# chrischoy/DeepGlobalRegistration

Hardware: AMD Instinct MI355X
Metric: pair registrations/sec (FCGF x2 + 1-NN + 6-D inlier net + gate + weighted Procrustes + SE(3) refinement) (higher is better)
Workload: dtype f32 results via 2 x f16 split operands (3 f16 MFMA products per MAC, f32 accumulate); k = 1 convs, kNN re-evaluation and registration in exact f32, SVD in f64

## Files before the change

### deepglobalregistration_amd/csrc/conv_os.hip

```cpp
#include <stdlib.h>

#include <type_traits>

#include "dgr_internal.h"
#include "split.h"

#ifdef DGR_OS_STAGE_CLK
__device__ unsigned long long dgr_os_stage_clk[8];
#define DGR_OS_CLK(i) do { if (threadIdx.x == 0) { const unsigned long long t_ = __builtin_amdgcn_s_memrealtime(); atomicAdd(&dgr_os_stage_clk[i], t_ - t_prev); t_prev = t_; } } while (0)
extern "C" int dgr_debug_os_stage_clk(unsigned long long *out8, int reset) {
  if (out8 && hipMemcpyFromSymbol(out8, HIP_SYMBOL(dgr_os_stage_clk), 8 * sizeof(unsigned long long)) != hipSuccess) return -1;
  if (reset) { unsigned long long z[8] = {0, 0, 0, 0, 0, 0, 0, 0}; if (hipMemcpyToSymbol(HIP_SYMBOL(dgr_os_stage_clk), z, sizeof(z)) != hipSuccess) return -1; }
  return 0;
}
#else
#define DGR_OS_CLK(i) do { } while (0)
#endif
struct ConvOsArgs {
  const float *in;
  float *out;
  const float *w16, *shift, *res;
  const uint4 *wb3;
  int64_t piece_stride;
  const int32_t *nbr, *n_out_dev;
  int64_t n_pad;
  int in_ld, in_relu, out_ld, out_relu, res_ld, res_relu;
  int cin, cout, nb16;
  const uint32_t *row_amax;
  float w_unscale;
  uint32_t *out_amax, *out_amax2;
};

template <int CP, int CS, int MB, int CK, int TM, int PM, int GW>
__global__ void __launch_bounds__(CS * 4 * (TM / 16 / GW)) sparse_conv_os(ConvOsArgs a) {
  constexpr bool BF3 = PM != 0;
  static_assert(PM == 0 || PM == 2, "arithmetic mode");
  constexpr int NP = PM == 0 ? 1 : 2;
  constexpr int GP = TM / 16;
  constexpr int NCW = CS / 16;
  constexpr int NWR = GP / GW;
  static_assert(GP % GW == 0, "groups per wave must divide the groups per tile");
  constexpr int NW = NCW * NWR;
  constexpr int THREADS = 64 * NW;
  constexpr int KV = 27;
  constexpr int PPT = CP / CK;
  constexpr int LDA = CK + 4, LDC = CS + 4;
  constexpr int C4K = CK / 4;
  constexpr int NCH = (TM * C4K + THREADS - 1) / THREADS;
  constexpr bool PIECE_GUARD = TM * C4K % THREADS != 0;
  constexpr int G = CK / 16;
  constexpr int GT = CP / 16;
  constexpr int KPW = (KV + NW - 1) / NW;
  constexpr int NGMAX = KV * ((MB / 16 + GP - 1) / GP * GP) + GP;
  static_assert(CP % CK == 0, "shape");
  constexpr int LDP = CK + 8;
  constexpr int PLANE = TM * LDP;
  constexpr int G32 = CK / 32;
  constexpr int ABYTES = BF3 ? 2 * NP * PLANE * 2 : 2 * TM * LDA * 4;
  __shared__ __attribute__((aligned(16))) char abuf[ABYTES];
  float (*As)[TM][LDA] = reinterpret_cast<float (*)[TM][LDA]>(abuf);
  unsigned short *Ps = reinterpret_cast<unsigned short *>(abuf);
  __shared__ __attribute__((aligned(16))) float acc_s[MB][LDC];
  __shared__ int in_idx[KV][MB];
  __shared__ float in_scale[PM == 2 ? KV : 1][MB];
  __shared__ unsigned char out_loc[KV][MB];
  __shared__ int cnt[KV];
  __shared__ int grp[NGMAX + GP];
  __shared__ int n_grp;

  const int tid = threadIdx.x;
  const int lane = tid & 63;
  const int wave = __builtin_amdgcn_readfirstlane(tid >> 6);
  const int cw = wave % NCW;
  const int rb0 = (wave / NCW) * GW;
  const int n_out = *a.n_out_dev;
  const int nblocks = (n_out + MB - 1) / MB;
  const int per = (nblocks + 7) >> 3;
  const int j = blockIdx.x >> 3;
  const int blk = (blockIdx.x & 7) * per + j;
  if (j >= per || blk >= nblocks) return;
  const int slice = blockIdx.y;
  const int64_t row0 = (int64_t)blk * MB;
#ifdef DGR_OS_STAGE_CLK
  unsigned long long t_prev = __builtin_amdgcn_s_memrealtime();
#endif

  if constexpr (PM == 2)
    for (int e = tid; e < KV * MB; e += THREADS) (&in_scale[0][0])[e] = 1.f;
  __syncthreads();
  {
    int v[KPW];
#pragma unroll
    for (int u = 0; u < KPW; ++u) {
      const int k = wave + u * NW;
      v[u] = (k < KV && lane < MB) ? a.nbr[(int64_t)k * a.n_pad + row0 + lane] : -1;
    }
#pragma unroll
    for (int u = 0; u < KPW; ++u) {
      const int k = wave + u * NW;
      if (k < KV) {
        const unsigned long long m = __ballot(v[u] >= 0);
        if (v[u] >= 0) {
          const int pos = __popcll(m & ((1ull << lane) - 1ull));
          in_idx[k][pos] = v[u];
          out_loc[k][pos] = (unsigned char)lane;
          if constexpr (PM == 2) in_scale[k][pos] = dgr_row_scale_of(a.row_amax[v[u]]);
        }
        if (lane == 0) cnt[k] = __popcll(m);
      }
    }
  }
  DGR_OS_CLK(0);
  for (int e = tid; e < MB * (CS / 4); e += THREADS) {
    const int r = e / (CS / 4), c = (e % (CS / 4)) * 4;
    f32x4 v = a.shift ? *reinterpret_cast<const f32x4 *>(a.shift + slice * CS + c) : f32x4{0.f, 0.f, 0.f, 0.f};
    if (a.res && row0 + r < n_out) {
      f32x4 x = *reinterpret_cast<const f32x4 *>(a.res + (row0 + r) * a.res_ld + slice * CS + c);
// ... 105 lines not shown
#pragma unroll
      for (int g = 0; g < G32; ++g) {
        const f16x8 ah = __builtin_bit_cast(f16x8, *reinterpret_cast<const uint4 *>(prow + 32 * g));
        const f16x8 am = __builtin_bit_cast(f16x8, *reinterpret_cast<const uint4 *>(prow + PLANE + 32 * g));
        const f16x8 wh = __builtin_bit_cast(f16x8, w[u].v[2 * g]), wm = __builtin_bit_cast(f16x8, w[u].v[2 * g + 1]);
        acc[u] = __builtin_amdgcn_mfma_f32_16x16x32_f16(wm, ah, acc[u], 0, 0, 0);
        acc[u] = __builtin_amdgcn_mfma_f32_16x16x32_f16(wh, am, acc[u], 0, 0, 0);
        acc[u] = __builtin_amdgcn_mfma_f32_16x16x32_f16(wh, ah, acc[u], 0, 0, 0);
      }
    }
  };
  if (NQ > 0) {
    gather(0);
#pragma unroll
    for (int u = 0; u < GW; ++u) wstep(0, u, w[u]);
    land(0);
    gather(NQ > 1 ? 1 : 0);
  }
  __syncthreads();

  for (int q = 0; q < NQ; ++q) {
    const int t = q / PPT, h = q % PPT;
    land(q + 1);
    gather(min(q + 2, NQ - 1));
    if (PPT == 1 || h == 0) {
#pragma unroll
      for (int u = 0; u < GW; ++u) acc[u] = f32x4{0.f, 0.f, 0.f, 0.f};
    }
#pragma unroll
    for (int u = 0; u < GW; ++u) {
      const int n_rows = __builtin_amdgcn_readfirstlane(grp[GP * t + rb0 + u]) >> 16;
      __builtin_amdgcn_sched_barrier(0);
      if (u == 0 || n_rows > 0) mfma_group(u, q & 1);
      wstep(q + 1, u, w[u]);
    }
    if (PPT == 1 || h == PPT - 1) {
#pragma unroll
      for (int u = 0; u < GW; ++u) {
        const int info = grp[GP * t + rb0 + u];
        if ((lane & 15) < (info >> 16)) {
          const int e = ((info >> 8) & 255) + (lane & 15);
          float *p = &acc_s[out_loc[info & 255][e]][16 * cw + 4 * (lane >> 4)];
          f32x4 v = *reinterpret_cast<f32x4 *>(p);
          if constexpr (PM == 2) {
            const float f = __builtin_bit_cast(float, 0x7f000000u - __builtin_bit_cast(uint32_t, in_scale[info & 255][e])) * a.w_unscale;
            v += acc[u] * f;
          } else {
            v += acc[u];
          }
          *reinterpret_cast<f32x4 *>(p) = v;
        }
      }
    }
    __syncthreads();
  }
  DGR_OS_CLK(2);
#ifdef DGR_OS_STAGE_CLK
  if (threadIdx.x == 0) { atomicAdd(&dgr_os_stage_clk[4], 1ull); atomicAdd(&dgr_os_stage_clk[5], (unsigned long long)NQ); }
#endif
  const float out_lo = a.out_relu ? 0.f : -__builtin_inff();
  static_assert(MB * (CS / 4) % THREADS == 0 || THREADS % (CS / 4) == 0, "row lanes stay inside a wave");
  for (int e0 = 0; e0 < MB * (CS / 4); e0 += THREADS) {
    const int e = e0 + tid;
    const bool live = e < MB * (CS / 4);
    const int r = live ? e / (CS / 4) : 0, c = (e % (CS / 4)) * 4;
    uint32_t mx = 0;
    if (live && row0 + r < n_out) {
      f32x4 v = *reinterpret_cast<const f32x4 *>(&acc_s[r][c]);
      v.x = fmaxf(v.x, out_lo); v.y = fmaxf(v.y, out_lo); v.z = fmaxf(v.z, out_lo); v.w = fmaxf(v.w, out_lo);
      *reinterpret_cast<f32x4 *>(a.out + (row0 + r) * a.out_ld + slice * CS + c) = v;
      mx = dgr_abs_max4(__builtin_bit_cast(i32x4, v));
    }
    if (a.out_amax || a.out_amax2) {
      mx = dgr_lane_max<CS / 4>(mx);
      if (live && (e % (CS / 4)) == 0 && row0 + r < n_out) {
        if (a.out_amax) atomicMax(a.out_amax + row0 + r, mx);
        if (a.out_amax2) atomicMax(a.out_amax2 + row0 + r, mx);
      }
    }
  }
  DGR_OS_CLK(3);
}

template <int CP, int CS, int MB, int CK, int TM>
static int launch_os(const ConvOsArgs &ka, int64_t n_out_cap, hipStream_t stream) {
  constexpr int GW = (MB >= 64 && CP <= 64) ? 1 : TM / 16;
  int64_t blocks = dgr_ceil_div(n_out_cap, MB);
  blocks = (blocks + 7) / 8 * 8;
  dim3 grid((unsigned)blocks, (unsigned)(ka.cout / CS));
  constexpr int threads = CS * 4 * (TM / 16 / GW);
  if (ka.wb3 && ka.row_amax)
    sparse_conv_os<CP, CS, MB, CK, TM, 2, GW><<<grid, threads, 0, stream>>>(ka);
  else
    sparse_conv_os<CP, CS, MB, CK, TM, 0, GW><<<grid, threads, 0, stream>>>(ka);
  DGR_LAUNCH_CHECK();
  return DGR_OK;
}

int dgr_conv_os_launch(const DgrConvOsLaunch &a, hipStream_t stream, const char **kernel_name) {
  if (a.dense) return dgr_conv_dense_launch(a, stream, kernel_name);
  if (a.up) return dgr_conv_up_launch(a, stream, kernel_name);
  DGR_REQUIRE(a.nbr && a.nbr->built && a.nbr->K == 27, "output-stationary conv: no neighbour table");
  DGR_REQUIRE((a.cin & 3) == 0 && (a.in_ld & 3) == 0 && (a.out_ld & 3) == 0 && (a.res == nullptr || (a.res_ld & 3) == 0),
              "output-stationary conv: channel counts and row strides must be multiples of 4");
  DGR_REQUIRE(a.cout % 32 == 0 && a.cin == a.cin_pad, "output-stationary conv: Cin = %d, Cout = %d must be multiples of 32",
              a.cin, a.cout);
  DGR_REQUIRE(a.n_in_cap > 0 && a.n_in_cap * (int64_t)a.in_ld < (1ll << 32) / 4 * 4,
              "output-stationary conv: input tensor beyond 32-bit element offsets");
  ConvOsArgs ka;
  ka.in = a.in; ka.out = a.out; ka.w16 = a.w16; ka.shift = a.shift; ka.res = a.res;
  ka.wb3 = dgr_exact_f32() ? nullptr : static_cast<const uint4 *>(a.wb3);
  ka.piece_stride = a.piece_stride;
  ka.row_amax = ka.wb3 ? a.row_amax : nullptr;
  ka.w_unscale = a.w_unscale;
  ka.out_amax = a.out_amax; ka.out_amax2 = a.out_amax2;
  DGR_REQUIRE(!ka.wb3 || ka.row_amax, "output-stationary conv: the split weights need the input rows' maxima");
  ka.nbr = a.nbr->nbr; ka.n_out_dev = a.n_out_dev; ka.n_pad = a.nbr->n_pad;
  ka.in_ld = a.in_ld; ka.in_relu = a.in_relu; ka.out_ld = a.out_ld; ka.out_relu = a.out_relu;
  ka.res_ld = a.res_ld; ka.res_relu = a.res_relu;
  ka.cin = a.cin; ka.cout = a.cout; ka.nb16 = a.cout / 16;
#define DGR_OS_TM 32
#define DGR_OS_MBBIG 64
#define DGR_STR2(x) #x
#define DGR_STR(x) DGR_STR2(x)
#define DGR_OS(CPV, CSV, MBV, CKV)                                                                      \
  do {                                                                                                  \
    constexpr int tm = (MBV) < DGR_OS_TM ? ((MBV) < 32 ? 32 : (MBV)) : DGR_OS_TM;                       \
    if (kernel_name) *kernel_name = ka.row_amax ? "sparse_conv_os<" #CPV ", " #CSV ", " DGR_STR(MBV) ", " DGR_STR(CKV) ", f16x2>"  \
                                                 : "sparse_conv_os<" #CPV ", " #CSV ", " DGR_STR(MBV) ", " DGR_STR(CKV) ", f32>"; \
    return launch_os<CPV, CSV, MBV, CKV, tm>(ka, a.n_out_cap, stream);                                  \
  } while (0)
  const int mb = a.rows_per_block;
  const bool narrow = a.cout == 32;
#define DGR_OS_MB(CPV, CKV)                                                 \
  do {                                                                      \
    if (narrow) { DGR_OS(CPV, 32, DGR_OS_MBBIG, CKV); }                     \
    else if (mb == 64) { DGR_OS(CPV, 64, DGR_OS_MBBIG, CKV); }              \
    else if (mb == 32) { DGR_OS(CPV, 64, 32, CKV); }                        \
    else { DGR_OS(CPV, 64, 16, CKV); }                                      \
  } while (0)
  const bool ck128 = a.phase_channels == 128;
  switch (a.cin_pad) {
    case 32: DGR_OS_MB(32, 32);
    case 64: DGR_OS_MB(64, 64);
    case 128: if (ck128) DGR_OS_MB(128, 128); else DGR_OS_MB(128, 64);
    case 256: if (ck128) DGR_OS_MB(256, 128); else DGR_OS_MB(256, 64);
    default: break;
  }
#undef DGR_OS_MB
#undef DGR_OS
  dgr_set_error("output-stationary conv: no instantiation for Cin (padded) %d", a.cin_pad);
  return DGR_EINVAL;
}
```

### deepglobalregistration_amd/csrc/dense_tile.h

```cpp
#pragma once
#include "dgr_internal.h"
#include "split.h"

struct DenseTileArgs {
  const float *in;
  float *out;
  const float *shift;
  const u32x4 *wb;
  int64_t piece_stride;
  const int32_t *nbr;
  int64_t n_pad;
  int in_ld, in_relu, out_ld, out_relu;
  float w_unscale;
  uint32_t in_bytes;
  const uint32_t *row_amax;
  uint32_t *out_amax, *out_amax2;
};

static inline int dgr_dense_tile_args(DenseTileArgs &ka, const DgrConvOsLaunch &a, const char *what) {
  DGR_REQUIRE(a.wbd && a.row_amax, "%s: needs the split weights in the dense-tile operand order and the input rows' maxima", what);
  DGR_REQUIRE((a.in_ld & 3) == 0 && (a.out_ld & 3) == 0 && (a.res == nullptr || (a.res_ld & 3) == 0),
              "%s: row strides must be multiples of 4", what);
  DGR_REQUIRE(a.n_in_cap > 0 && dgr_fits_32bit_offsets(a.n_in_cap, a.in_ld), "%s: input tensor beyond 2 GB", what);
  ka.in = a.in; ka.out = a.out; ka.shift = a.shift;
  ka.wb = static_cast<const u32x4 *>(a.wbd); ka.piece_stride = a.piece_stride;
  ka.nbr = a.nbr->nbr; ka.n_pad = a.nbr->n_pad;
  ka.in_ld = a.in_ld; ka.in_relu = a.in_relu; ka.out_ld = a.out_ld; ka.out_relu = a.out_relu;
  ka.row_amax = a.row_amax; ka.out_amax = a.out_amax; ka.out_amax2 = a.out_amax2;
  ka.w_unscale = a.w_unscale;
  ka.in_bytes = (uint32_t)(a.n_in_cap * (int64_t)a.in_ld * 4);
  return DGR_OK;
}

template <int RG, int S>
struct DenseTileRows { f32x4 raw[RG][S][2]; uint32_t mx[RG]; int nv[RG]; };

template <int RG, int S, bool PS, class NbrOf>
__device__ __forceinline__ void dense_tile_request(DenseTileRows<RG, S> &g, const NbrOf &nbr_of, const int &lane,
                                                   const __amdgpu_buffer_rsrc_t &in_rsrc, const DenseTileArgs &a,
                                                   uint32_t col_bytes) {
#pragma unroll
  for (int rg = 0; rg < RG; ++rg) {
    const int n = nbr_of(rg);
    const int ne = max(n, 0);
    const uint32_t off = n >= 0 ? (uint32_t)n * (uint32_t)((PS ? 32 * S : a.in_ld) * 4) + col_bytes + 16u * (lane & 3) : a.in_bytes;
    const uint32_t mv = a.row_amax[ne];
#pragma unroll
    for (int s = 0; s < S; ++s) {
      if constexpr (PS) {
        g.raw[rg][s][0] = __builtin_bit_cast(f32x4, __builtin_amdgcn_raw_buffer_load_b128(in_rsrc, off + 64 * s, 0, 0));
        g.raw[rg][s][1] = __builtin_bit_cast(f32x4, __builtin_amdgcn_raw_buffer_load_b128(in_rsrc, off + 64 * S + 64 * s, 0, 0));
      } else {
        g.raw[rg][s][0] = __builtin_bit_cast(f32x4, __builtin_amdgcn_raw_buffer_load_b128(in_rsrc, off + 128 * s, 0, 0));
        g.raw[rg][s][1] = __builtin_bit_cast(f32x4, __builtin_amdgcn_raw_buffer_load_b128(in_rsrc, off + 128 * s + 64, 0, 0));
      }
    }
    g.mx[rg] = mv;
    g.nv[rg] = n;
  }
}

template <bool PS>
__device__ __forceinline__ void dense_tile_operand(f32x4 c0, f32x4 c1, int from, int relu_lo, float sx, f16x8 &bh, f16x8 &bm) {
  i32x4 hw, mw;
  if constexpr (PS) {
    hw = __builtin_bit_cast(i32x4, c0);
    mw = __builtin_bit_cast(i32x4, c1);
  } else {
    dgr_split2_x8(__builtin_bit_cast(i32x4, c0), __builtin_bit_cast(i32x4, c1), relu_lo, sx, hw, mw);
  }
#pragma unroll
  for (int d = 0; d < 4; ++d) {
    hw[d] = __builtin_amdgcn_ds_bpermute(from, hw[d]);
    mw[d] = __builtin_amdgcn_ds_bpermute(from, mw[d]);
  }
  bh = __builtin_bit_cast(f16x8, hw);
  bm = __builtin_bit_cast(f16x8, mw);
}

template <int RG, int S>
__device__ __forceinline__ void dense_tile_mfma(f32x4 (&tmp)[RG], f16x8 wh, f16x8 wm, const f16x8 (&bh)[RG][S],
                                                const f16x8 (&bm)[RG][S], int s) {
#pragma unroll
  for (int rg = 0; rg < RG; ++rg) tmp[rg] = __builtin_amdgcn_mfma_f32_16x16x32_f16(wm, bh[rg][s], tmp[rg], 0, 0, 0);
#pragma unroll
  for (int rg = 0; rg < RG; ++rg) tmp[rg] = __builtin_amdgcn_mfma_f32_16x16x32_f16(wh, bm[rg][s], tmp[rg], 0, 0, 0);
#pragma unroll
  for (int rg = 0; rg < RG; ++rg) tmp[rg] = __builtin_amdgcn_mfma_f32_16x16x32_f16(wh, bh[rg][s], tmp[rg], 0, 0, 0);
}

template <int NCB>
__device__ __forceinline__ uint32_t dense_tile_store_row(f32x4 (&total)[NCB], int64_t row, float *out, int out_ld, int out_relu, int lq,
                                                         bool want_max, uint32_t *out_amax, uint32_t *out_amax2) {
  const float out_lo = out_relu ? 0.f : -__builtin_inff();
  uint32_t mx = 0;
#pragma unroll
  for (int cb = 0; cb < NCB; ++cb) {
    f32x4 v = total[cb];
    v.x = fmaxf(v.x, out_lo); v.y = fmaxf(v.y, out_lo); v.z = fmaxf(v.z, out_lo); v.w = fmaxf(v.w, out_lo);
    total[cb] = v;
    if (row >= 0) {
      if (out) *reinterpret_cast<f32x4 *>(out + row * out_ld + 16 * cb) = v;
      mx = max(mx, dgr_abs_max4(__builtin_bit_cast(i32x4, v)));
    }
  }
  if (want_max) {
    mx = dgr_lane_max<4, 16>(mx);
    if (lq == 0 && row >= 0) {
      if (out_amax) atomicMax(out_amax + row, mx);
      if (out_amax2) atomicMax(out_amax2 + row, mx);
    }
  }
  return mx;
}
```

### deepglobalregistration_amd/csrc/dgr_internal.h

```cpp
#pragma once
#include <hip/hip_runtime.h>
#include <stdint.h>
#include <stdio.h>
#include <stdlib.h>
#include <string>
#include <vector>

#include "../../include/dgr_hip.h"

void dgr_set_error(const char *fmt, ...);

#define DGR_HIP_CHECK(expr)                                                                  \
  do {                                                                                       \
    hipError_t _e = (expr);                                                                  \
    if (_e != hipSuccess) {                                                                  \
      dgr_set_error("%s:%d: %s failed: %s", __FILE__, __LINE__, #expr, hipGetErrorString(_e)); \
      return DGR_EHIP;                                                                       \
    }                                                                                        \
  } while (0)

#define DGR_CHECK(expr)          \
  do {                           \
    int _r = (expr);             \
    if (_r != DGR_OK) return _r; \
// ... 98 lines not shown
  DgrNbrTable nsame[4];
  DgrNbrTable ndown[3];
  DgrNbrTable nup[3];
  DgrCoordMap cm[4];
  DgrHalfBuckets hb[4];
  DgrKernelMap same[4];
  DgrKernelMap conv1;
  DgrKernelMap down[3];
  int32_t *overflow = nullptr;
};

int dgr_build_maps(DgrArena &arena, const int32_t *coords, int64_t N, int D, int conv1_ks,
                   DgrMapSet *ms, hipStream_t stream, bool skip_conv1_map = false, bool lean = false,
                   bool nbr_tables = false);
int dgr_nbr_counts(const DgrNbrTable &t, const int32_t *n_out_dev, int64_t counts[27]);
int dgr_conv1_probe(DgrArena &arena, const DgrCoordMap &cm, int ks, const float *in, int in_ld, int cin,
                    const float *w_tiled, const float *shift, float *out, int out_ld, int32_t *pair_count,
                    hipStream_t stream, const float *w_compact = nullptr, const char **kernel_name = nullptr,
                    uint32_t *out_amax = nullptr);
constexpr int32_t DGR_ROW_DROPPED = -1, DGR_ROW_PENDING = -2;
int dgr_unique_rows(DgrArena &arena, const int32_t *keys, int64_t n, int nc, const int32_t *state, int32_t *held,
                    int32_t *first_flag, int32_t *rank, int32_t *n_unique_dev, int32_t **table_out, uint32_t *mask_out,
                    hipStream_t stream);
int dgr_exclusive_scan_i32(DgrArena &arena, const int32_t *in, int32_t *out, int64_t n,
                           int32_t *total_out, hipStream_t stream);
constexpr int DGR_SCAN_MAX = 24;
int dgr_exclusive_scan_multi(DgrArena &arena, int count, const int32_t *const *in, int32_t *const *out, const int64_t *n,
                             int32_t *const *total_out, hipStream_t stream);

struct DgrConvLaunch {
  const float *in;
  int in_ld;
  int in_relu;
  float *out;
  int out_ld;
  float *y;
  const float *shift;
  const float *w;
  int cin, cin_pad, cout, cout_pad, K;
  const int32_t *pair_in, *pair_out, *tile_ptr, *rule_ptr;
  const int4 *tile_desc;
  const int32_t *n_rows_dev;
  int64_t tile_bound;
  int l2_normalize = 0;
  unsigned long long *clk = nullptr;
};
int dgr_conv_launch(const DgrConvLaunch &a, int num_cus, hipStream_t stream, const char **kernel_name = nullptr);
struct DgrSplitRows {
  unsigned char *planes = nullptr;
  float *scale = nullptr;
  int channels = 0;
};
bool dgr_conv_wide_supported(int cin_pad, int cin, int cout);
int dgr_conv_wide_launch(const DgrConvLaunch &a, const DgrSplitRows &in, const void *wb, int64_t piece_stride,
                         float w_unscale, int num_cus, hipStream_t stream, const char **kernel_name = nullptr);
int dgr_row_amax(const float *in, int in_ld, int cin, int relu, const int32_t *n_dev, int64_t n_cap, uint32_t *out,
                 hipStream_t stream);
int dgr_split_rows(const float *in, int in_ld, int relu, const int32_t *n_dev, int64_t n_cap, const DgrSplitRows &out,
                   hipStream_t stream);
int dgr_reduce_rows(const float *y, int cout, const int32_t *ptr, const int32_t *pos, const int32_t *n_dev,
                    int64_t n_cap, float *out, int out_ld, const float *shift, const float *res, int res_ld,
                    int res_relu, hipStream_t stream, const DgrSplitRows *split = nullptr, int out_relu = 0);
int dgr_conv_small_cin(const float *in, int in_ld, int in_relu, int cin, const float *w_tiled, const float *w_quad,
                       const float *shift, const DgrKernelMap &km, const int32_t *n_out_dev, int64_t n_out_cap, float *out,
                       int out_ld, hipStream_t stream);
struct DgrConvOsLaunch {
  const float *in; int in_ld, in_relu;
  float *out; int out_ld, out_relu;
  const float *w16, *shift;
  const void *wb3; int64_t piece_stride;
  const void *wbd = nullptr;
  const uint32_t *row_amax = nullptr; float w_unscale = 1.f;
  uint32_t *out_amax = nullptr, *out_amax2 = nullptr;
  int64_t n_in_cap = 0;
  const float *res; int res_ld, res_relu;
  int rows_per_block;
  int phase_channels = 64;
  const DgrNbrTable *nbr;
  const int32_t *n_out_dev;
  int64_t n_out_cap;
  int cin, cin_pad, cout;
  bool dense = false;
  bool up = false;
  const unsigned char *in_dsplit = nullptr;
  unsigned char *out_dsplit = nullptr;
};
inline bool dgr_fits_32bit_offsets(int64_t rows, int64_t ld) { return rows * ld * 4 < (1ll << 31); }
int dgr_conv_os_launch(const DgrConvOsLaunch &a, hipStream_t stream, const char **kernel_name = nullptr);
bool dgr_conv_dense_supported(int cin, int cin_pad, int cout);
int dgr_conv_dense_launch(const DgrConvOsLaunch &a, hipStream_t stream, const char **kernel_name = nullptr);
bool dgr_conv_up_supported(int cin, int cin_pad, int cout);
int dgr_conv_up_launch(const DgrConvOsLaunch &a, hipStream_t stream, const char **kernel_name = nullptr);
int dgr_l2_normalize_rows(const float *in, int in_ld, float *out, int out_ld, int c, int relu,
                          const int32_t *n_dev, int64_t n_cap, hipStream_t stream);

struct DgrBatchOutputs {
  const void *ptr[5] = {nullptr, nullptr, nullptr, nullptr, nullptr};
  int64_t numel[5] = {0, 0, 0, 0, 0};
  uint64_t generation = 0;
};

struct DgrEventPool {
  std::vector<hipEvent_t> ev;
  size_t used = 0;
  hipEvent_t next();
  void release();
};

struct dgr_ctx {
  int device = 0;
  int num_cus = 256;
  DgrArena arena;
  bool profiling = false;
  float stage_ms[9] = {0, 0, 0, 0, 0, 0, 0, 0, 0};
  int64_t conv_launches = 0;
  DgrBatchOutputs last;
  std::vector<double> last_T64;
  DgrEventPool events;
  std::vector<std::pair<hipEvent_t, hipEvent_t>> conv_spans, gemm_spans, map3_spans, map6_spans;
  std::vector<float> conv_span_ms, gemm_span_ms;
  std::vector<unsigned long long *> conv_clks;
  std::vector<float> conv_clk_us;
  std::vector<const char *> conv_kinds;
  int32_t *flag_dev = nullptr;
  hipEvent_t wait_ev = nullptr;
  long last_wait_ns = 0;
  double batch_ns_per_row = 0;
  double pairs_ns_per_row = 0;
  unsigned char *pin = nullptr;
  size_t pin_bytes = 0;
  hipStream_t part_stream = nullptr;
  int all_cus = 256;
};

int dgr_ctx_pinned(dgr_ctx *ctx, size_t bytes, unsigned char **out);
int dgr_flag_error(int32_t flag);

int dgr_ctx_wait(dgr_ctx *ctx, hipStream_t stream, long predicted_ns = 0);

int dgr_resunet_forward_impl(dgr_ctx *ctx, dgr_net *net, const int32_t *coords, const float *feats,
                             int64_t N, float *out, hipStream_t stream);
int dgr_ctx_collect_profile(dgr_ctx *ctx);
void dgr_ctx_begin_profile(dgr_ctx *ctx);

int dgr_knn1_batch_impl(dgr_ctx *ctx, const float *F0, const int64_t *off0, const float *F1, const int64_t *off1,
                        int npairs, int C, int squared, int64_t *idx_out, float *dist_out, hipStream_t stream);
int dgr_knn1_impl(dgr_ctx *ctx, const float *F0, int64_t N0, const float *F1, int64_t N1, int C,
                  int squared, int64_t *idx_out, float *dist_out, hipStream_t stream);
int dgr_inlier_inputs_impl(const int32_t *coords0, const float *xyz0, int64_t N0,
                           const int32_t *coords1, const float *xyz1, const int64_t *idx1,
                           int feature_type, int32_t *coords6, float *feats, hipStream_t stream);
int dgr_icp_impl(dgr_ctx *ctx, const float *src, int64_t N0, const float *dst, int64_t N1, double max_dist,
                 const double *T_init, int max_iter, double rel_fitness, double rel_rmse, double *T_out,
                 double *stats_out, hipStream_t stream);
int dgr_ransac_impl(dgr_ctx *ctx, const float *X, const float *Y, int64_t N, double max_dist, int64_t num_hypotheses,
                    uint32_t seed, double *T_out, double *stats_out, hipStream_t stream);
struct DgrIcpJob {
  const float *src = nullptr, *dst = nullptr;
  int64_t N0 = 0, N1 = 0;
  double max_dist = 0;
  int nblocks = 0;
  void *st = nullptr;
  double *P = nullptr, *sorted = nullptr, *partial = nullptr;
  int32_t ncell = 0;
  double host_state[64];
};
int dgr_icp_begin(dgr_ctx *ctx, const float *src, int64_t N0, const float *dst, int64_t N1, double max_dist,
                  const double *T_init_dev , DgrIcpJob *job, hipStream_t stream);
int dgr_icp_run(dgr_ctx *ctx, DgrIcpJob *job, int max_iter, double rel_fitness, double rel_rmse, hipStream_t stream);
void dgr_icp_finish(const DgrIcpJob *job, double *T_out, double *stats_out);
constexpr int DGR_RANSAC_RESULT_DOUBLES = 19;
// ... 14 lines not shown
```

### deepglobalregistration_amd/csrc/net.hip

```cpp
#include <math.h>
#include <stdlib.h>
#include <string.h>

#include <algorithm>
#include <map>
#include <memory>
#include <string>

#include "dgr_internal.h"

static const int CH[5] = {0, 32, 64, 128, 256};
static const int TR[5] = {0, 64, 64, 64, 128};
static constexpr float BN_EPS = 1e-5f;

struct DgrLayer {
  std::string name;
  int K, cin, cout, cin_pad, cout_pad;
  float *w = nullptr;
  float *w16 = nullptr;
  void *w16b = nullptr;
  void *w16d = nullptr;
  int64_t w16b_piece = 0;
  float *wc = nullptr;
  float *wq = nullptr;
// ... 421 lines not shown
  hipStream_t stream;
  DgrMapSet ms;
  bool prof;
  bool l2_next = false;

  float *ybuf = nullptr;

  int conv(int li, const Tensor &in, const DgrKernelMap *km, bool swapped, int lvl_in, int lvl_out,
           const Tensor &out, const Tensor *res) {
    const DgrLayer &L = net->W->layers[li];
    const DgrCoordMap &cin_map = ms.cm[lvl_in], &cout_map = ms.cm[lvl_out];
    DgrConvLaunch a;
    a.in = in.ptr; a.in_ld = in.ld; a.in_relu = in.relu;
    a.out = out.ptr; a.out_ld = out.ld;
    a.y = ybuf; a.shift = L.shift;
    a.w = L.w;
    a.cin = L.cin; a.cin_pad = L.cin_pad; a.cout = L.cout; a.cout_pad = L.cout_pad; a.K = L.K;
    if (km && ms.use_nbr) {
      a.pair_in = a.pair_out = a.tile_ptr = a.rule_ptr = nullptr;
      a.tile_desc = nullptr; a.n_rows_dev = nullptr; a.tile_bound = 0;
    } else if (km) {
      a.pair_in = swapped ? km->pair_out : km->pair_in;
      a.pair_out = swapped ? km->pair_in : km->pair_out;
      a.tile_ptr = km->tile_ptr; a.rule_ptr = km->rule_ptr; a.tile_desc = km->tile_desc;
      a.n_rows_dev = nullptr;
      a.tile_bound = km->pair_cap / DGR_TILE_M + km->K;
      DGR_REQUIRE(km->K == L.K, "layer %s: kernel volume mismatch", L.name.c_str());
      DGR_REQUIRE(!swapped || km->in_ptr, "layer %s: map has no in-major CSR", L.name.c_str());
    } else {
      DGR_REQUIRE(res == nullptr, "identity conv with residual not supported");
      a.pair_in = a.pair_out = a.tile_ptr = a.rule_ptr = nullptr;
      a.tile_desc = nullptr;
      a.n_rows_dev = cout_map.n_dev;
      a.tile_bound = dgr_ceil_div(cout_map.n_cap, DGR_TILE_M);
      a.l2_normalize = l2_next ? 1 : 0;
      l2_next = false;
    }
    hipEvent_t e0 = nullptr, em = nullptr, e1 = nullptr;
    if (prof) {
      e0 = ctx->events.next(); em = ctx->events.next(); e1 = ctx->events.next();
      if (!e0 || !em || !e1) return DGR_EHIP;
      DGR_HIP_CHECK(hipEventRecord(e0, stream));
    }
    if (km && ms.use_nbr) {
      const DgrNbrTable *t = nullptr;
      for (int l = 0; l < 4; ++l)
        if (km == &ms.same[l]) t = &ms.nsame[l];
      for (int l = 0; l < 3; ++l)
        if (km == &ms.down[l]) t = swapped ? &ms.nup[l] : &ms.ndown[l];
      DGR_REQUIRE(t && t->built && L.w16, "layer %s: no neighbour table / 16x16 weights", L.name.c_str());
      DgrConvOsLaunch o;
      o.in = in.ptr; o.in_ld = in.ld; o.in_relu = in.relu;
      o.out = out.ptr; o.out_ld = out.ld; o.out_relu = out.relu;
      o.rows_per_block = lvl_out <= 1 ? 64 : lvl_out == 2 ? (L.cin_pad >= 128 ? 64 : 32) : 16;
      o.phase_channels = (L.cin_pad >= 256 || (L.cin_pad == 128 && lvl_out >= 2)) ? 128 : 64;
      if (const char *e = getenv(lvl_out == 2 ? "DGR_OS_MB2" : lvl_out == 3 ? "DGR_OS_MB3" : "DGR_OS_MB01")) o.rows_per_block = atoi(e);
      if (const char *e = getenv("DGR_OS_CK")) o.phase_channels = atoi(e);
      o.w16 = L.w16; o.shift = L.shift;
      o.wb3 = L.w16b; o.piece_stride = L.w16b_piece;
      o.wbd = L.w16d;
      o.w_unscale = L.w_unscale; o.n_in_cap = cin_map.n_cap;
      if (L.w16b && !dgr_exact_f32()) {
        o.row_amax = in.amax;
        if (!o.row_amax) {
          uint32_t *mx;
          DGR_ALLOC(mx, ctx->arena, uint32_t, cin_map.n_cap);
          DGR_CHECK(dgr_row_amax(in.ptr, in.ld, L.cin, in.relu, cin_map.n_dev, cin_map.n_cap, mx, stream));
          o.row_amax = mx;
        }
      }
      o.out_amax = out.amax; o.out_amax2 = out.amax2;
      o.res = res ? res->ptr : nullptr; o.res_ld = res ? res->ld : 0; o.res_relu = res ? res->relu : 0;
      o.nbr = t; o.n_out_dev = cout_map.n_dev; o.n_out_cap = cout_map.n_cap;
      o.cin = L.cin; o.cin_pad = L.cin_pad; o.cout = L.cout;
      static const bool os_lists = getenv("DGR_OS_LISTS") != nullptr;
      bool same_stride = false;
      for (int l = 0; l < 4; ++l) same_stride = same_stride || t == &ms.nsame[l];
      o.dense = same_stride && o.row_amax && o.wbd && !os_lists && dgr_conv_dense_supported(L.cin, L.cin_pad, L.cout) &&
                dgr_fits_32bit_offsets(cin_map.n_cap, in.ld);
      DGR_REQUIRE(o.dense || (!in.dsplit_only && !out.dsplit_only), "layer %s: dense split rows outside the dense-tile kernel", L.name.c_str());
      static const bool no_up = getenv("DGR_NO_UP") != nullptr;
      o.up = swapped && !o.dense && !no_up && !os_lists && o.row_amax && o.wbd && t->perm && res == nullptr &&
             dgr_conv_up_supported(L.cin, L.cin_pad, L.cout) && dgr_fits_32bit_offsets(cin_map.n_cap, in.ld);
      if (o.dense) {
        o.in_dsplit = in.dsplit;
        o.out_dsplit = out.dsplit;
        if (out.dsplit_only) o.out = nullptr;
      }
      const char *kname = "sparse_conv_os";
      DGR_CHECK(dgr_conv_os_launch(o, stream, &kname));
      if (prof) {
        DGR_HIP_CHECK(hipEventRecord(e1, stream));
        ctx->conv_spans.push_back({e0, e1});
        ctx->gemm_spans.push_back({e0, e1});
        ctx->conv_kinds.push_back(kname);
      }
      LayerRun &r = net->runs[li];
      r = LayerRun();
      r.os = true;
      r.os_launch = o;
      r.nbr = *t;
      r.os_launch.nbr = &r.nbr;
      r.n_in = cin_map.n_dev; r.n_out = cout_map.n_dev; r.K = L.K;
      r.n_out_cap = cout_map.n_cap;
      return DGR_OK;
    }
    const bool small_cin = km && !swapped && !res && L.cin <= 8 && L.cout == 32 && L.cin_pad == 8;
    const char *kname = (L.cin == 6 && L.wq) ? "conv_cin6_quad_kernel" : L.cin == 1 ? "conv_small_cin_row_kernel" : "conv_small_cin_kernel";
    unsigned long long *clk = nullptr;
    const bool wide = L.wb && km;
    if (small_cin)
      DGR_CHECK(dgr_conv_small_cin(in.ptr, in.ld, in.relu, L.cin, L.w, L.wq, L.shift, *km, cout_map.n_dev, cout_map.n_cap,
                                   out.ptr, out.ld, stream));
    else if (wide) {
      DGR_REQUIRE(in.split.planes, "layer %s: the wide-layer kernel needs its input as split rows", L.name.c_str());
      if (prof) {
        DGR_ALLOC(a.clk, ctx->arena, unsigned long long, 2);
        DGR_HIP_CHECK(hipMemsetAsync(a.clk, 0xff, sizeof(unsigned long long), stream));
        DGR_HIP_CHECK(hipMemsetAsync(a.clk + 1, 0, sizeof(unsigned long long), stream));
        clk = a.clk;
      }
      DGR_CHECK(dgr_conv_wide_launch(a, in.split, L.wb, L.wb_piece, L.w_unscale, ctx->num_cus, stream, &kname));
    } else
      DGR_CHECK(dgr_conv_launch(a, ctx->num_cus, stream, &kname));
    if (prof) DGR_HIP_CHECK(hipEventRecord(em, stream));
    DGR_REQUIRE(!out.split.planes || (km && !small_cin), "layer %s: only a reduction can write split rows", L.name.c_str());
    if (km && !small_cin)
      DGR_CHECK(dgr_reduce_rows(ybuf, L.cout, swapped ? km->in_ptr : km->out_ptr, swapped ? km->in_pos : km->out_pos,
                                cout_map.n_dev, cout_map.n_cap, out.split_only ? nullptr : out.ptr, out.ld, L.shift, res ? res->ptr : nullptr,
                                res ? res->ld : 0, res ? res->relu : 0, stream, out.split.planes ? &out.split : nullptr,
                                out.relu));
    if (prof) {
      DGR_HIP_CHECK(hipEventRecord(e1, stream));
      ctx->conv_spans.push_back({e0, e1});
      ctx->gemm_spans.push_back({e0, em});
      ctx->conv_kinds.push_back(kname);
      ctx->conv_clks.resize(ctx->conv_spans.size(), nullptr);
      ctx->conv_clks.back() = clk;
    }
    LayerRun &r = net->runs[li];
    a.clk = nullptr;
    r.launch = a;
    r.split_in = wide ? in.split : DgrSplitRows();
    r.split_out = out.split;
    r.out_relu = out.relu;
    r.split_only = out.split_only;
    r.has_reduce = km != nullptr;
    r.small_cin = small_cin;
    if (km) r.km = *km;
    if (km) {
      r.red_ptr = swapped ? km->in_ptr : km->out_ptr;
      r.red_pos = swapped ? km->in_pos : km->out_pos;
    }
    r.n_out_cap = cout_map.n_cap;
    r.res = res ? res->ptr : nullptr; r.res_ld = res ? res->ld : 0; r.res_relu = res ? res->relu : 0;
    r.rule_ptr = km ? km->rule_ptr : nullptr;
    r.n_in = cin_map.n_dev; r.n_out = cout_map.n_dev; r.K = L.K;
    return DGR_OK;
  }
};

int dgr_resunet_forward_impl(dgr_ctx *ctx, dgr_net *net, const int32_t *coords, const float *feats,
                             int64_t N, float *out, hipStream_t stream) {
  DgrArena &A = ctx->arena;
  Fwd f;
  f.ctx = ctx; f.net = net; f.stream = stream; f.prof = ctx->profiling;
// ... 473 lines not shown
```

Before: 401.8.

## Add list-free output-stationary conv path using dense-tile MFMA gathers

Adds a new output-stationary sparse conv mode for Cin 128/256 that skips the per-offset neighbour lists. It stages the 27-offset neighbour table in shared memory, gathers input rows with buffer loads in the dense-tile split operand format, and keeps a register ring of split weights that is prefetched ahead of the MFMAs. The goal is to cut gather and list overhead on the strided (non-same-stride) downsampling convs. It is enabled by default for eligible non-swapped layers with per-level rows-per-block choices, and it adds DPP lane swizzling to the operand builder plus extra register pressure.

```diff
diff --git a/deepglobalregistration_amd/csrc/conv_os.hip b/deepglobalregistration_amd/csrc/conv_os.hip
--- a/deepglobalregistration_amd/csrc/conv_os.hip
+++ b/deepglobalregistration_amd/csrc/conv_os.hip
@@ -2,8 +2,7 @@
 
 #include <type_traits>
 
-#include "dgr_internal.h"
-#include "split.h"
+#include "dense_tile.h"
 
 #ifdef DGR_OS_STAGE_CLK
 __device__ unsigned long long dgr_os_stage_clk[8];
@@ -29,10 +28,11 @@
   const uint32_t *row_amax;
   float w_unscale;
   uint32_t *out_amax, *out_amax2;
+  uint32_t in_bytes;
 };
 
 template <int CP, int CS, int MB, int CK, int TM, int PM, int GW>
-__global__ void __launch_bounds__(CS * 4 * (TM / 16 / GW)) sparse_conv_os(ConvOsArgs a) {
+__device__ __forceinline__ void conv_os_lists(const ConvOsArgs &a) {
   constexpr bool BF3 = PM != 0;
   static_assert(PM == 0 || PM == 2, "arithmetic mode");
   constexpr int NP = PM == 0 ? 1 : 2;
@@ -304,6 +304,169 @@
   DGR_OS_CLK(3);
 }
 
+#ifndef DGR_OS_TILES_DEPTH
+#define DGR_OS_TILES_DEPTH 1
+#endif
+#ifndef DGR_OS_TILES_WD
+#define DGR_OS_TILES_WD 8
+#endif
+template <int CIN, int MB, int RG>
+__device__ __forceinline__ void conv_os_tiles(const ConvOsArgs &a) {
+  constexpr int KV = 27;
+  constexpr int NCB = 4;
+  constexpr int NCH = CIN / 64;
+  constexpr int S_T = CIN / 32;
+  constexpr int WAVES = MB / (16 * RG);
+  constexpr int THREADS = 64 * WAVES;
+  constexpr int NST = 2 * NCB;
+  constexpr int NIT = KV * NCH;
+  constexpr int DEPTH = DGR_OS_TILES_DEPTH;
+  constexpr int WD = DGR_OS_TILES_WD;
+  static_assert(NST % WD == 0, "the weight ring turns a whole number of times per (offset, chunk)");
+  static_assert(CIN % 64 == 0 && MB % (16 * RG) == 0 && NIT % DEPTH == 0, "shape");
+  __shared__ int nbr_s[KV][MB];
+
+  const int tid = threadIdx.x, lane = tid & 63;
+  const int wave = __builtin_amdgcn_readfirstlane(tid >> 6);
+  const int slice = blockIdx.y;
+  const int n_out = *a.n_out_dev;
+  const int nblocks = (n_out + MB - 1) / MB;
+  const int per = (nblocks + 7) >> 3;
+  const int j = blockIdx.x >> 3;
+  const int blk = (blockIdx.x & 7) * per + j;
+  if (j >= per || blk >= nblocks) return;
+  const int64_t row0 = (int64_t)blk * MB;
+
+  for (int e = tid; e < KV * MB; e += THREADS) {
+    const int k = e / MB, r = e - k * MB;
+    nbr_s[k][r] = (row0 + r < n_out) ? a.nbr[(int64_t)k * a.n_pad + row0 + r] : -1;
+  }
+  u32x4 rh[WD], rm[WD];
+  const u32x4 *wph = reinterpret_cast<const u32x4 *>(a.wb3) + lane, *wpm = wph + a.piece_stride;
+  auto wreq = [&](int g, int i) {
+    const int gc = min(g, NIT * NST - 1);
+    const int it = gc / NST, jj = gc - it * NST;
+    const int k = it / NCH, ch = it - k * NCH;
+    const int64_t frag = ((int64_t)k * S_T + 2 * ch + (jj & 1)) * a.nb16 + slice * NCB + (jj >> 1);
+    rh[i] = wph[frag * 64];
+    rm[i] = wpm[frag * 64];
+  };
+  const int lr = lane & 15, lq = lane >> 4;
+  f32x4 total[RG][NCB];
+#pragma unroll
+  for (int cb = 0; cb < NCB; ++cb) {
+    const f32x4 sh = a.shift ? *reinterpret_cast<const f32x4 *>(a.shift + 64 * slice + 16 * cb + 4 * lq) : f32x4{0.f, 0.f, 0.f, 0.f};
+#pragma unroll
+    for (int rg = 0; rg < RG; ++rg) {
+      f32x4 v = sh;
+      const int64_t row = row0 + (wave * RG + rg) * 16 + lr;
+      if (a.res && row < n_out) {
+        f32x4 x = *reinterpret_cast<const f32x4 *>(a.res + row * a.res_ld + 64 * slice + 16 * cb + 4 * lq);
+        if (a.res_relu) { x.x = fmaxf(x.x, 0.f); x.y = fmaxf(x.y, 0.f); x.z = fmaxf(x.z, 0.f); x.w = fmaxf(x.w, 0.f); }
+        v += x;
+      }
+      total[rg][cb] = v;
+    }
+  }
+  __syncthreads();
+
+  DenseTileArgs d = {};
+  d.in_ld = a.in_ld; d.in_bytes = a.in_bytes; d.row_amax = a.row_amax;
+  const __amdgpu_buffer_rsrc_t in_rsrc = __builtin_amdgcn_make_buffer_rsrc(const_cast<float *>(a.in), 0, a.in_bytes, 0x00020000);
+  using Rows = DenseTileRows<RG, 2>;
+  auto gather = [&](int it, Rows &g) {
+    const int k = it / NCH, ch = it - k * NCH;
+    dense_tile_request<RG, 2, false>(g, [&](int rg) { return nbr_s[k][(wave * RG + rg) * 16 + (lane >> 2)]; }, lane, in_rsrc,
+                                     d, 256u * ch);
+  };
+  Rows gR[DEPTH];
+#pragma unroll
+  for (int i = 0; i < DEPTH; ++i) gather(i, gR[i]);
+#pragma unroll
+  for (int i = 0; i < WD; ++i) wreq(i, i);
+  const int relu_lo = a.in_relu ? 0 : (int)0x80000000;
+  const bool odd = lane & 1;
+  const int from = 4 * (4 * (lane & 15) + ((lane >> 3) & 2) + (lane >> 5));
+
+  f32x4 tmp[NCB][RG];
+  auto body = [&](int it, Rows &gA) {
+    const int ch = it % NCH;
+    f16x8 bh[RG][2], bm[RG][2];
+    float fold[RG];
+#pragma unroll
+    for (int rg = 0; rg < RG; ++rg) {
+      const float sx = gA.nv[rg] >= 0 ? dgr_row_scale_of(gA.mx[rg]) : 0.f;
+      const float fl = sx != 0.f ? dgr_inv_pow2(sx) * a.w_unscale : 0.f;
+      fold[rg] = __builtin_bit_cast(float, __builtin_amdgcn_ds_bpermute(16 * (lane & 15), __builtin_bit_cast(int, fl)));
+#pragma unroll
+      for (int s = 0; s < 2; ++s)
+        dense_tile_operand<false, true>(gA.raw[rg][s][0], gA.raw[rg][s][1], from, relu_lo, sx, bh[rg][s], bm[rg][s], odd);
+    }
+    __builtin_amdgcn_sched_barrier(0);
+    gather(min(it + DEPTH, NIT - 1), gA);
+    __builtin_amdgcn_sched_barrier(0);
+    if (ch == 0) {
+#pragma unroll
+      for (int rg = 0; rg < RG; ++rg)
+#pragma unroll
+        for (int cb = 0; cb < NCB; ++cb) tmp[cb][rg] = f32x4{0.f, 0.f, 0.f, 0.f};
+    }
+#pragma unroll
+    for (int cb = 0; cb < NCB; ++cb) {
+#pragma unroll
+      for (int s = 0; s < 2; ++s) {
+        const int jj = cb * 2 + s;
+        const f16x8 wh = __builtin_bit_cast(f16x8, rh[jj % WD]);
+        const f16x8 wm = __builtin_bit_cast(f16x8, rm[jj % WD]);
+        dense_tile_mfma(tmp[cb], wh, wm, bh, bm, s);
+        wreq(it * NST + jj + WD, jj % WD);
+        __builtin_amdgcn_sched_barrier(0);
+      }
+    }
+    if (ch == NCH - 1) {
+#pragma unroll
+      for (int rg = 0; rg < RG; ++rg)
+#pragma unroll
+        for (int cb = 0; cb < NCB; ++cb) total[rg][cb] += tmp[cb][rg] * fold[rg];
+    }
+  };
+#pragma unroll 1
+  for (int it = 0; it < NIT; it += DEPTH) {
+#pragma unroll
+    for (int i = 0; i < DEPTH; ++i) body(it + i, gR[i]);
+  }
+
+#pragma unroll
+  for (int rg = 0; rg < RG; ++rg) {
+    const int64_t r = row0 + (wave * RG + rg) * 16 + lr;
+    dense_tile_store_row(total[rg], r < n_out ? r : -1, a.out + 64 * slice + 4 * lq, a.out_ld, a.out_relu, lq,
+                         a.out_amax || a.out_amax2, a.out_amax, a.out_amax2);
+  }
+}
+
+constexpr int dgr_os_threads(int CS, int MB, int TM, int GW) { return TM ? CS * 4 * (TM / 16 / GW) : 64 * (MB / (16 * GW)); }
+
+template <int CP, int CS, int MB, int CK, int TM, int PM, int GW>
+__global__ void __launch_bounds__(dgr_os_threads(CS, MB, TM, GW), TM ? 1 : 2) sparse_conv_os(ConvOsArgs a) {
+  if constexpr (TM == 0) {
+    static_assert(CS == 64 && CK == 64 && PM == 2, "list-free mode: 64-column slices, 64-channel chunks, split operands");
+    conv_os_tiles<CP, MB, GW>(a);
+  } else {
+    conv_os_lists<CP, CS, MB, CK, TM, PM, GW>(a);
+  }
+}
+
+template <int CP, int MB>
+static int launch_os_tiles(const ConvOsArgs &ka, int64_t n_out_cap, hipStream_t stream) {
+  constexpr int RG = 2;
+  int64_t blocks = dgr_ceil_div(n_out_cap, MB);
+  blocks = (blocks + 7) / 8 * 8;
+  dim3 grid((unsigned)blocks, (unsigned)(ka.cout / 64));
+  sparse_conv_os<CP, 64, MB, 64, 0, 2, RG><<<grid, dgr_os_threads(64, MB, 0, RG), 0, stream>>>(ka);
+  DGR_LAUNCH_CHECK();
+  return DGR_OK;
+}
+
 template <int CP, int CS, int MB, int CK, int TM>
 static int launch_os(const ConvOsArgs &ka, int64_t n_out_cap, hipStream_t stream) {
   constexpr int GW = (MB >= 64 && CP <= 64) ? 1 : TM / 16;
@@ -317,6 +480,10 @@
     sparse_conv_os<CP, CS, MB, CK, TM, 0, GW><<<grid, threads, 0, stream>>>(ka);
   DGR_LAUNCH_CHECK();
   return DGR_OK;
+}
+
+bool dgr_conv_os_tiles_supported(int cin, int cin_pad, int cout) {
+  return cin == cin_pad && (cin == 128 || cin == 256) && cout % 64 == 0 && cout >= 64;
 }
 
 int dgr_conv_os_launch(const DgrConvOsLaunch &a, hipStream_t stream, const char **kernel_name) {
@@ -341,6 +508,22 @@
   ka.in_ld = a.in_ld; ka.in_relu = a.in_relu; ka.out_ld = a.out_ld; ka.out_relu = a.out_relu;
   ka.res_ld = a.res_ld; ka.res_relu = a.res_relu;
   ka.cin = a.cin; ka.cout = a.cout; ka.nb16 = a.cout / 16;
+  ka.in_bytes = 0;
+  if (a.tiles) {
+    DGR_REQUIRE(ka.wb3 && ka.row_amax && dgr_conv_os_tiles_supported(a.cin, a.cin_pad, a.cout),
+                "output-stationary conv, list-free mode: Cin = %d, Cout = %d not built, or no split weights", a.cin, a.cout);
+    DGR_REQUIRE(dgr_fits_32bit_offsets(a.n_in_cap, a.in_ld), "output-stationary conv, list-free mode: input tensor beyond 2 GB");
+    ka.in_bytes = (uint32_t)(a.n_in_cap * (int64_t)a.in_ld * 4);
+#define DGR_OS_TILES(CPV, MBV)                                                                  \
+    if (a.cin == CPV && a.rows_per_block == MBV) {                                                \
+      if (kernel_name) *kernel_name = "sparse_conv_os<" #CPV ", 64, " #MBV ", 64, 0, 2, 2>";      \
+      return launch_os_tiles<CPV, MBV>(ka, a.n_out_cap, stream);                                  \
+    }
+    DGR_OS_TILES(128, 128) DGR_OS_TILES(128, 64) DGR_OS_TILES(256, 128) DGR_OS_TILES(256, 64)
+#undef DGR_OS_TILES
+    dgr_set_error("output-stationary conv, list-free mode: no instantiation for Cin %d, %d rows per workgroup", a.cin, a.rows_per_block);
+    return DGR_EINVAL;
+  }
 #define DGR_OS_TM 32
 #define DGR_OS_MBBIG 64
 #define DGR_STR2(x) #x
diff --git a/deepglobalregistration_amd/csrc/dense_tile.h b/deepglobalregistration_amd/csrc/dense_tile.h
--- a/deepglobalregistration_amd/csrc/dense_tile.h
+++ b/deepglobalregistration_amd/csrc/dense_tile.h
@@ -60,14 +60,24 @@
   }
 }
 
-template <bool PS>
-__device__ __forceinline__ void dense_tile_operand(f32x4 c0, f32x4 c1, int from, int relu_lo, float sx, f16x8 &bh, f16x8 &bm) {
+template <bool PS, bool NAT = false>
+__device__ __forceinline__ void dense_tile_operand(f32x4 c0, f32x4 c1, int from, int relu_lo, float sx, f16x8 &bh, f16x8 &bm,
+                                                   bool odd = false) {
   i32x4 hw, mw;
   if constexpr (PS) {
     hw = __builtin_bit_cast(i32x4, c0);
     mw = __builtin_bit_cast(i32x4, c1);
   } else {
     dgr_split2_x8(__builtin_bit_cast(i32x4, c0), __builtin_bit_cast(i32x4, c1), relu_lo, sx, hw, mw);
+  }
+  if constexpr (NAT) {
+#pragma unroll
+    for (int d = 0; d < 2; ++d) {
+      const int gh = __builtin_amdgcn_mov_dpp(odd ? hw[d] : hw[2 + d], 0xB1, 0xf, 0xf, true);
+      const int gm = __builtin_amdgcn_mov_dpp(odd ? mw[d] : mw[2 + d], 0xB1, 0xf, 0xf, true);
+      hw[d] = odd ? gh : hw[d]; hw[2 + d] = odd ? hw[2 + d] : gh;
+      mw[d] = odd ? gm : mw[d]; mw[2 + d] = odd ? mw[2 + d] : gm;
+    }
   }
 #pragma unroll
   for (int d = 0; d < 4; ++d) {
diff --git a/deepglobalregistration_amd/csrc/dgr_internal.h b/deepglobalregistration_amd/csrc/dgr_internal.h
--- a/deepglobalregistration_amd/csrc/dgr_internal.h
+++ b/deepglobalregistration_amd/csrc/dgr_internal.h
@@ -204,11 +204,13 @@
   int cin, cin_pad, cout;
   bool dense = false;
   bool up = false;
+  bool tiles = false;
   const unsigned char *in_dsplit = nullptr;
   unsigned char *out_dsplit = nullptr;
 };
 inline bool dgr_fits_32bit_offsets(int64_t rows, int64_t ld) { return rows * ld * 4 < (1ll << 31); }
 int dgr_conv_os_launch(const DgrConvOsLaunch &a, hipStream_t stream, const char **kernel_name = nullptr);
+bool dgr_conv_os_tiles_supported(int cin, int cin_pad, int cout);
 bool dgr_conv_dense_supported(int cin, int cin_pad, int cout);
 int dgr_conv_dense_launch(const DgrConvOsLaunch &a, hipStream_t stream, const char **kernel_name = nullptr);
 bool dgr_conv_up_supported(int cin, int cin_pad, int cout);
diff --git a/deepglobalregistration_amd/csrc/net.hip b/deepglobalregistration_amd/csrc/net.hip
--- a/deepglobalregistration_amd/csrc/net.hip
+++ b/deepglobalregistration_amd/csrc/net.hip
@@ -527,6 +527,13 @@
       static const bool no_up = getenv("DGR_NO_UP") != nullptr;
       o.up = swapped && !o.dense && !no_up && !os_lists && o.row_amax && o.wbd && t->perm && res == nullptr &&
              dgr_conv_up_supported(L.cin, L.cin_pad, L.cout) && dgr_fits_32bit_offsets(cin_map.n_cap, in.ld);
+      static const bool no_tiles = getenv("DGR_OS_NO_TILES") != nullptr;
+      o.tiles = !swapped && !o.dense && !no_tiles && !os_lists && o.row_amax && o.wb3 &&
+                dgr_conv_os_tiles_supported(L.cin, L.cin_pad, L.cout) && dgr_fits_32bit_offsets(cin_map.n_cap, in.ld);
+      if (o.tiles) {
+        o.rows_per_block = lvl_out <= 2 ? 128 : 64;
+        if (const char *e = getenv(lvl_out <= 2 ? "DGR_OS_TILES_MB2" : "DGR_OS_TILES_MB3")) o.rows_per_block = atoi(e);
+      }
       if (o.dense) {
         o.in_dsplit = in.dsplit;
         o.out_dsplit = out.dsplit;
```

Result: faster. 408.3, median of 6 (+1.6%).
